# 3dhumangan/3DHumanGAN

Hardware: NVIDIA H100
Metric: images_per_sec_G_fwd_512x512 (higher is better)
Workload: dtype f32 (bf16x3 split on wgmma, fp32 accumulate)

## Files before the change

### 3dhumangan_b200/abi.py

```python
from __future__ import annotations

import ctypes
import os
from ctypes import c_char_p, c_double, c_float, c_int, c_long, c_size_t, c_void_p

import torch

_HERE = os.path.dirname(os.path.abspath(__file__))
LIB_PATH = os.path.join(_HERE, "lib3dhg_sm90a.so")
_lib = None

SIGNATURES = {
    "hg_last_error": (c_char_p, []),
    "hg_abi_version": (c_int, []),
    "hg_check_device": (c_int, []),
    "hg_packed_weight_bytes": (c_size_t, [c_int, c_int, c_int]),
    "hg_pack_weight": (c_int, [c_void_p, c_int, c_int, c_int, c_void_p, c_float, c_int, c_void_p, c_size_t, c_void_p]),
    "hg_vertex_ik": (c_int, [c_void_p, c_void_p, c_int, c_int, c_void_p, c_void_p]),
    "hg_knn_padded": (c_int, [c_int]),
    "hg_knn_prep": (c_int, [c_void_p, c_int, c_int, c_void_p, c_void_p, c_void_p]),
    "hg_geo_features": (c_int, [c_void_p] * 14 + [c_int] * 6 + [c_float, c_int] + [c_void_p] * 6),
    "hg_sample_fine": (c_int, [c_void_p, c_int, c_void_p, c_void_p, c_void_p, c_float, c_int] + [c_void_p] * 4 + [c_int] * 4
                       + [c_void_p] * 3),
    "hg_merge_samples": (c_int, [c_void_p] * 4 + [c_int] * 3 + [c_void_p] * 4),
    "hg_iso_workspace_bytes": (c_size_t, [c_int, c_int, c_int]),
    "hg_iso_count": (c_int, [c_void_p, c_int, c_int, c_int, c_float, c_void_p, c_size_t, c_void_p, c_void_p]),
    "hg_iso_emit": (c_int, [c_void_p, c_int, c_int, c_int] + [c_float] * 5 + [c_void_p, c_size_t, ctypes.c_longlong]
                    + [c_void_p] * 4),
    "hg_spade_conv": (c_int, [c_void_p, c_long, c_void_p, c_void_p, c_void_p, c_long] + [c_void_p] * 12 + [c_int] * 7 + [c_void_p]),
    "hg_bn_finalize": (c_int, [c_void_p, c_double, c_void_p, c_void_p, c_void_p, c_void_p, c_void_p, c_int, c_float, c_float,
                               c_void_p, c_int, c_int, c_void_p, c_void_p, c_void_p]),
    "hg_synth_input": (c_int, [c_void_p, c_void_p, c_void_p, c_void_p, c_int, c_int, c_int, c_void_p, c_void_p, c_int, c_void_p]),
    "hg_render_weight_blob_bytes": (c_size_t, []),
    "hg_render_mlp": (c_int, [c_void_p] * 12 + [c_int] * 4 + [c_float] + [c_int] * 4 + [c_void_p]),
    "hg_spade_bwd_dgrad": (c_int, [c_void_p, c_void_p, c_long, c_void_p, c_void_p, c_void_p, c_void_p] + [c_int] * 5 + [c_void_p]),
    "hg_spade_bwd_wgrad_workspace_bytes": (c_size_t, []),
    "hg_spade_bwd_wgrad": (c_int, [c_void_p, c_void_p, c_long, c_void_p, c_void_p, c_void_p, c_void_p] + [c_int] * 5 + [c_void_p]),
    "hg_spade_bwd_combine": (c_int, [c_void_p, c_void_p, c_long] + [c_void_p] * 7 + [c_int] * 4 + [c_void_p]),
    "hg_conv1x1_blocked": (c_int, [c_void_p, c_int, c_void_p, c_void_p, c_void_p] + [c_int] * 4 + [c_void_p]),
    "hg_conv1x1_blocked_bwd": (c_int, [c_void_p] * 7 + [c_int, c_float, c_int, c_int, c_void_p, c_void_p, c_void_p, c_int]
                               + [c_int] * 4 + [c_void_p]),
    "hg_act_conv1x1_blocked": (c_int, [c_void_p, c_void_p, c_void_p, c_int, c_void_p, c_void_p, c_void_p] + [c_int] * 4 + [c_void_p]),
    "hg_act_wgrad_blocked": (c_int, [c_void_p, c_void_p, c_void_p, c_long, c_int, c_void_p, c_int, c_void_p, c_void_p, c_void_p]
                             + [c_int] * 5 + [c_void_p]),
    "hg_render_heads": (c_int, [c_void_p] * 8 + [c_int, c_int, c_void_p]),
    "hg_render_heads_bwd": (c_int, [c_void_p] * 6 + [c_int, c_int, c_void_p]),
    "hg_render_composite": (c_int, [c_void_p] * 7 + [c_int, c_int, c_int, c_float, c_int, c_int, c_int, c_void_p]),
    "hg_blocked_conv_wide": (c_int, [c_void_p] * 4 + [c_int, c_float] + [c_void_p] * 9 + [c_int] * 4 + [c_void_p]),
    "hg_render_composite_bwd": (c_int, [c_void_p] * 9 + [c_int, c_int, c_int, c_float, c_int, c_int, c_int, c_void_p]),
    "hg_wgrad_blocked": (c_int, [c_void_p, c_void_p, c_long, c_int, c_void_p, c_void_p, c_void_p, c_void_p] + [c_int] * 5 + [c_void_p]),
    "hg_spade_a1": (c_int, [c_void_p, c_long, c_void_p, c_void_p] + [c_int] * 5 + [c_void_p]),
    "hg_spade_pixel_pre": (c_int, [c_void_p, c_long, c_void_p, c_void_p, c_void_p] + [c_int] * 4 + [c_void_p]),
    "hg_spade_pixel_mod_bwd": (c_int, [c_void_p, c_void_p, c_long, c_void_p, c_void_p, c_void_p, c_void_p] + [c_int] * 4 + [c_void_p]),
    "hg_bilinear_adjoint": (c_int, [c_void_p, c_void_p, c_long] + [c_int] * 5 + [c_void_p]),
    "hg_conv2d_wgrad_workspace_bytes": (c_size_t, []),
    "hg_conv2d_wgrad_taps": (c_int, [c_void_p] * 5 + [c_int] * 10 + [c_void_p, c_void_p, c_int, c_void_p]),
    "hg_conv2d_wgrad_layer_workspace_bytes": (c_size_t, [c_int] * 6),
    "hg_conv2d_wgrad_layer": (c_int, [c_void_p] * 5 + [c_size_t] + [c_int] * 7 + [c_void_p]),
    "hg_synth_input_bwd": (c_int, [c_void_p] * 5 + [c_int] * 4 + [c_void_p, c_void_p, c_void_p]),
    "hg_bias_act": (c_int, [c_void_p, c_void_p, c_void_p, c_long, c_int, c_int, c_int, c_float, c_float, c_float, c_void_p]),
    "hg_bias_act_grad": (c_int, [c_void_p] * 6 + [c_long, c_int, c_int, c_int, c_int, c_float, c_float, c_float, c_void_p]),
    "hg_resample2x": (c_int, [c_void_p, c_void_p, c_long, c_int, c_int, c_int, c_float, c_void_p]),
    "hg_upfirdn2d": (c_int, [c_void_p, c_void_p, c_void_p] + [c_int] * 14 + [c_float, c_void_p]),
    "hg_upfirdn2d_sep2": (c_int, [c_void_p, c_void_p, c_void_p, c_long] + [c_int] * 9 + [c_float, c_void_p]),
    "hg_conv2d": (c_int, [c_void_p, c_int, c_void_p, c_int] + [c_int] * 6 + [c_void_p, c_int, c_int, c_void_p, c_void_p, c_int,
                              c_void_p, c_int, c_void_p]),
    "hg_pool_add": (c_int, [c_void_p, c_int, c_void_p, c_int, c_void_p, c_long, c_int, c_int, c_void_p]),
    "hg_dense": (c_int, [c_void_p, c_void_p, c_void_p, c_void_p, c_int, c_int, c_int, c_void_p]),
    "hg_linear": (c_int, [c_void_p, c_int, c_int, c_int, c_void_p, c_int, c_int, c_void_p, c_void_p, c_int, c_int, c_void_p]),
    "hg_conv3x3_wgrad_halo_workspace_bytes": (ctypes.c_size_t, []),
    "hg_conv3x3_wgrad_halo": (c_int, [c_void_p] * 5 + [c_int] * 10 + [c_void_p, c_void_p, c_int, c_void_p]),
    "hg_label_histogram": (c_int, [c_void_p, c_long, c_int, c_void_p, c_void_p]),
    "hg_seg_ce_coef": (c_int, [c_void_p, c_void_p, c_int, c_double, c_void_p, c_void_p]),
    "hg_seg_ce": (c_int, [c_void_p] * 6 + [c_int, c_int, c_long, c_void_p]),
    "hg_image_loss": (c_int, [c_void_p] * 6 + [c_int, c_long, c_int, c_float, c_void_p]),
    "hg_latent_pool_gather": (c_int, [c_void_p, c_long, c_int, c_void_p, c_int, c_void_p, c_void_p]),
    "hg_latent_pool_grad": (c_int, [c_void_p, c_void_p, c_int, c_int, c_long, c_void_p, c_void_p]),
    "hg_latent_loss": (c_int, [c_void_p, c_void_p, c_int, c_int, c_float, c_void_p, c_void_p, c_void_p, c_void_p]),
    "hg_vgg_input": (c_int, [c_void_p, c_int, c_int, c_int, c_int, c_void_p, c_void_p, c_void_p, c_int, c_int, c_void_p]),
    "hg_vgg_input_adjoint": (c_int, [c_void_p, c_int, c_int, c_int, c_void_p, c_void_p, c_int, c_int, c_int, c_void_p]),
    "hg_maxpool2x2": (c_int, [c_void_p, c_void_p, c_long, c_int, c_int, c_void_p]),
    "hg_vgg_level_bwd": (c_int, [c_void_p] * 4 + [c_float, c_void_p, c_long, c_int, c_int, c_void_p]),
    "hg_smooth_l1": (c_int, [c_void_p, c_void_p, c_long, c_void_p, c_void_p, c_void_p]),
    "hg_conv2d_general": (c_int, [c_void_p] + [c_int] * 9 + [c_void_p, c_int, c_int, c_void_p, c_void_p, c_int, c_int, c_int,
                                                             c_void_p]),
    "hg_pool3x3": (c_int, [c_void_p] + [c_int] * 7 + [c_void_p, c_int, c_int, c_void_p]),
    "hg_global_avgpool": (c_int, [c_void_p, c_long, c_int, c_void_p, c_void_p]),
    "hg_feature_moments": (c_int, [c_void_p, c_int, c_int, c_void_p, c_void_p, c_void_p]),
    "hg_row_sqnorms": (c_int, [c_void_p, c_int, c_int, c_void_p, c_void_p]),
    "hg_knn_radii": (c_int, [c_void_p, c_void_p, c_int, c_int, c_int, c_void_p, c_void_p]),
    "hg_ball_coverage": (c_int, [c_void_p, c_void_p, c_void_p, c_int, c_void_p, c_void_p, c_void_p, c_int, c_int, c_void_p, c_void_p,
                                 c_void_p, c_void_p]),
    "hg_kid_workspace_bytes": (c_size_t, [c_int, c_int]),
    "hg_kid": (c_int, [c_void_p, c_int, c_void_p, c_int, c_int, c_void_p, c_void_p, c_int, c_int, c_void_p, c_void_p, c_size_t,
                       c_void_p]),
    "hg_mt_entry_bytes": (c_int, []),
    "hg_mt_chunk_bytes": (c_int, []),
    "hg_mt_chunk_elems": (c_int, []),
    "hg_mt_grad_norm": (c_int, [c_void_p, c_void_p, c_int, c_float, c_void_p, c_void_p, c_void_p]),
    "hg_mt_adam": (c_int, [c_void_p, c_void_p, c_int, c_void_p, c_void_p, c_int, c_float, c_int, c_void_p]),
    "hg_smpl_shape_blocks": (c_int, [c_int]),
    "hg_smpl_shape": (c_int, [c_void_p] * 6 + [c_int] * 4 + [c_void_p]),
    "hg_smpl_pose": (c_int, [c_void_p, c_int, c_void_p, c_int] + [c_void_p] * 6 + [c_int, c_int, c_void_p]),
    "hg_smpl_skin": (c_int, [c_void_p, c_long, c_void_p, c_void_p, c_int, c_void_p, c_long, c_void_p, c_void_p, c_int, c_int, c_int, c_void_p]),
    "hg_raster_project": (c_int, [c_void_p, c_void_p, c_void_p, c_float, c_void_p, c_int, c_int, c_void_p]),
    "hg_raster_faces": (c_int, [c_void_p, c_void_p] + [c_int] * 5 + [c_void_p, c_void_p]),
    "hg_raster_resolve": (c_int, [c_void_p] * 5 + [c_int] * 5 + [c_void_p] * 6),
    "hg_spectral_entry_bytes": (c_int, []),
    "hg_spectral_norm": (c_int, [c_void_p, c_int, c_int, c_int, c_void_p, c_int, c_float, c_void_p]),
}


def lib():
    global _lib
    if _lib is None:
        if not os.path.exists(LIB_PATH):
            raise RuntimeError(
# ... 495 lines not shown
```

### 3dhumangan_b200/csrc/render.cu

```cuda
#include "common.cuh"
#include "wgmma.cuh"

namespace hg {

constexpr int kRH = 256;
constexpr int kRenThreads = 384;
constexpr int kRenStages = 2;
constexpr uint32_t kRA = 128 * 128;
constexpr uint32_t kRB = 256 * 128;
constexpr int kFilmLayers = 7;
constexpr int kWeightStages = 60;
constexpr int kRayOut = 260;
constexpr int kScr = 65;

struct RenderArgs {
  const float* rec;
  const float* z_vals;
  const float* noise;
  const float* film;
  const uint8_t* wblob;
  const float* w_sigma;
  const float* w_rgb;
  const float* b_feat;
  const float* heads_b;
  float* ray_out;
  float* weights_out;
  float* raw_out;
  int B, R, S;
  float noise_std;
  int white_back, last_back, clamp_softplus;
};

struct RenSmem {
  uint8_t* a_hi;
  uint8_t* a_lo;
  uint8_t* b_st;
  float* film;
  float* w_sigma;
  float* w_rgb;
  float* b_feat;
  float* part;
  float* tr;
  float* wgt;
  float* zs;
  float* rayw;
  uint64_t* bars;
};
constexpr uint32_t kRenFloats = kFilmLayers * 2 * kRH + kRH + 3 * kRH + kRH + 128 * 4 + 4 * 128;
constexpr uint32_t kRenSmemBytes = 8 * kRA + kRenStages * kRB + kRenFloats * 4 + 16 * 8 + 1024;

__device__ __forceinline__ RenSmem ren_carve(uint8_t* raw) {
  uint8_t* s = reinterpret_cast<uint8_t*>((reinterpret_cast<uintptr_t>(raw) + 1023) & ~uintptr_t(1023));
  RenSmem m;
  m.a_hi = s;
  m.a_lo = s + 4 * kRA;
  m.b_st = s + 8 * kRA;
  float* f = reinterpret_cast<float*>(m.b_st + kRenStages * kRB);
  m.film = f; f += kFilmLayers * 2 * kRH;
  m.w_sigma = f; f += kRH;
  m.w_rgb = f; f += 3 * kRH;
  m.b_feat = f; f += kRH;
  m.part = f; f += 128 * 4;
  m.tr = f; f += 128;
  m.wgt = f; f += 128;
  m.zs = f; f += 128;
  m.rayw = f; f += 128;
  m.bars = reinterpret_cast<uint64_t*>(f);
  return m;
}
enum { RB_FULL = 0 , RB_EMPTY = 2  };

__device__ __forceinline__ void ren_rows_barrier() { named_barrier(1, 256); }

__device__ __forceinline__ float sin_reduced(float t) {
  const float y = t * 0.15915494309189535f;
  const float k = (y + 12582912.f) - 12582912.f;
  float r = fmaf(-k, 6.2831854820251465f, t);
  r = fmaf(-k, -1.7484555314695172e-07f, r);
  return __sinf(r);
}

__device__ __forceinline__ float2 sin_reduced2(float2 t) {
  const float2 y = fmul2(t, make_float2(0.15915494309189535f, 0.15915494309189535f));
  const float2 big = make_float2(12582912.f, 12582912.f), nbig = make_float2(-12582912.f, -12582912.f);
  const float2 k = fadd2(fadd2(y, big), nbig);
  float2 r = ffma2(k, make_float2(-6.2831854820251465f, -6.2831854820251465f), t);
  r = ffma2(k, make_float2(1.7484555314695172e-07f, 1.7484555314695172e-07f), r);
  return make_float2(__sinf(r.x), __sinf(r.y));
}

template <bool kSplit>
__device__ __forceinline__ void store_a2(uint8_t* tile_hi, uint8_t* tile_lo, uint32_t row, uint32_t k, float x0, float x1) {
  uint32_t h, l;
  split_bf16x2(x0, x1, h, l);
  const uint32_t off = sw128_offset(row, k);
  asm volatile("st.shared.b32 [%0], %1;" ::"r"(smem_u32(tile_hi) + off), "r"(h));
  if (kSplit) asm volatile("st.shared.b32 [%0], %1;" ::"r"(smem_u32(tile_lo) + off), "r"(l));
}

__device__ __forceinline__ void stash_store(float* slot, const float (&d)[128]) {
  const uint32_t base = static_cast<uint32_t>(__cvta_generic_to_local(slot));
#pragma unroll
  for (int i = 0; i < 128; i += 4)
    asm volatile("st.local.v4.f32 [%0], {%1, %2, %3, %4};" ::"r"(base + i * 4), "f"(d[i]), "f"(d[i + 1]), "f"(d[i + 2]), "f"(d[i + 3])
                 : "memory");
}
__device__ __forceinline__ float4 stash_load4(const float* slot, int i) {
  float4 v;
  asm volatile("ld.local.v4.f32 {%0, %1, %2, %3}, [%4];" : "=f"(v.x), "=f"(v.y), "=f"(v.z), "=f"(v.w)
               : "r"(static_cast<uint32_t>(__cvta_generic_to_local(slot)) + i * 4)
               : "memory");
  return v;
}

template <int kPasses, int kHead, bool kStash = false>
__device__ __forceinline__ void film_epilogue(const RenSmem& m, const float (&d)[128], const float* stash, int layer, int g, int t) {
  uint32_t F = smem_u32(m.film + (layer * 2 + 0) * kRH);
  uint32_t P = smem_u32(m.film + (layer * 2 + 1) * kRH);
  opaque(F);
  opaque(P);
  float dots[2][3] = {{0.f, 0.f, 0.f}, {0.f, 0.f, 0.f}};
#pragma unroll
  for (int j = 0; j < 32; ++j) {
    const int c = frag_col(t, j, 0);
    float f2[2], p2[2];
    asm("ld.shared.v2.f32 {%0, %1}, [%2];" : "=f"(f2[0]), "=f"(f2[1]) : "r"(F + c * 4));
    asm("ld.shared.v2.f32 {%0, %1}, [%2];" : "=f"(p2[0]), "=f"(p2[1]) : "r"(P + c * 4));
    float v[4] = {d[4 * j], d[4 * j + 1], d[4 * j + 2], d[4 * j + 3]};
    if (kStash) {
      const float4 q = stash_load4(stash, 4 * j);
      v[0] = q.x; v[1] = q.y; v[2] = q.z; v[3] = q.w;
    }
#pragma unroll
    for (int i = 0; i < 2; ++i) {
      const float2 x = sin_reduced2(ffma2(make_float2(f2[0], f2[1]), make_float2(v[2 * i], v[2 * i + 1]),
                                          make_float2(p2[0], p2[1])));
      if (kHead == 1) dots[i][0] = fmaf(x.y, m.w_sigma[c + 1], fmaf(x.x, m.w_sigma[c], dots[i][0]));
      if (kHead == 2) {
#pragma unroll
        for (int h = 0; h < 3; ++h) dots[i][h] = fmaf(x.y, m.w_rgb[h * kRH + c + 1], fmaf(x.x, m.w_rgb[h * kRH + c], dots[i][h]));
      }
      const int kc = c >> 6;
      store_a2<kPasses == 3>(m.a_hi + kc * kRA, m.a_lo + kc * kRA, g * 64 + frag_row(t, i), c & 63, x.x, x.y);
    }
  }
  if (kHead != 0) {
#pragma unroll
    for (int i = 0; i < 2; ++i) {
#pragma unroll
      for (int h = 0; h < 3; ++h) {
        if (kHead == 1 && h > 0) break;
        float v = dots[i][h];
        v += __shfl_xor_sync(0xffffffffu, v, 1);
        v += __shfl_xor_sync(0xffffffffu, v, 2);
        if ((t & 3) == 0) m.part[(g * 64 + frag_row(t, i)) * 4 + (kHead == 1 ? 0 : 1 + h)] = v;
      }
    }
  }
  fence_proxy_async_smem();
  named_barrier(2 + g, 128);
}

template <int kPasses>
__global__ void __launch_bounds__(kRenThreads, 1) render_mlp_kernel(RenderArgs a) {
  extern __shared__ uint8_t smem_raw[];
  const RenSmem m = ren_carve(smem_raw);
  const int warp = threadIdx.x >> 5, lane = threadIdx.x & 31;
  for (int i = threadIdx.x; i < kRH; i += blockDim.x) {
    m.w_sigma[i] = a.w_sigma[i];
    m.b_feat[i] = a.b_feat[i];
  }
  for (int i = threadIdx.x; i < 3 * kRH; i += blockDim.x) m.w_rgb[i] = a.w_rgb[i];
  if (threadIdx.x == 0) {
    for (int i = 0; i < kRenStages; ++i) {
      mbar_init(m.bars + RB_FULL + i, 1);
      mbar_init(m.bars + RB_EMPTY + i, 2);
    }
    fence_mbar_init();
  }
  __syncthreads();

  const int S = a.S;
  const int rpt = 128 / S;
  const int tiles_per_img = (a.R + rpt - 1) / rpt;
  const int num_tiles = a.B * tiles_per_img;
  const int my_tiles = (num_tiles - static_cast<int>(blockIdx.x) + static_cast<int>(gridDim.x) - 1) / static_cast<int>(gridDim.x);
  const long N = static_cast<long>(a.R) * S;

  if (warp < 8) {
    regs_inc<kMmaRegs>();
    const int g = warp >> 2, t = threadIdx.x & 127;
    const int tid = threadIdx.x;
    float d[128];
    __align__(16) float stash[128];
    uint32_t st = 0, ph = 0;
    uint32_t prev = ~0u;
    auto stage = [&](uint32_t a_tile, uint32_t a_tile2, bool two, bool accumulate) {
      mbar_wait(m.bars + RB_FULL + st, ph);
      acc_fence(d);
      wgmma_fence();
      const uint32_t bt = smem_u32(m.b_st + st * kRB);
      wg_k64<256>(d, a_tile, bt, accumulate);
      if (two) wg_k64<256>(d, a_tile2, bt, true);
      wgmma_commit();
      wgmma_wait<1>();
      acc_fence(d);
      if (prev != ~0u && t == 0) mbar_arrive(m.bars + RB_EMPTY + prev);
      prev = st;
      if (++st == kRenStages) { st = 0; ph ^= 1; }
    };
    auto layer = [&](int k0, int nk, bool accumulate) {
      for (int kc = k0; kc < k0 + nk; ++kc) {
        const uint32_t ahi = smem_u32(m.a_hi + kc * kRA) + g * 64 * 128, alo = smem_u32(m.a_lo + kc * kRA) + g * 64 * 128;
        stage(ahi, alo, kPasses == 3, accumulate || kc > k0);
        if (kPasses == 3) stage(ahi, ahi, false, true);
      }
      wgmma_wait<0>();
      acc_fence(d);
      if (t == 0) mbar_arrive(m.bars + RB_EMPTY + prev);
      prev = ~0u;
    };
    int cur_b = -1;
    for (int it = 0; it < my_tiles; ++it) {
      const int tile = blockIdx.x + it * gridDim.x;
      const int b = tile / tiles_per_img;
      const int ray0 = (tile % tiles_per_img) * rpt;
      if (b != cur_b) {
        ren_rows_barrier();
        for (int i = tid; i < kFilmLayers * 2 * kRH; i += 256)
          m.film[i] = a.film[static_cast<long>(b) * kFilmLayers * 2 * kRH + i];
        cur_b = b;
        ren_rows_barrier();
      }
      {
        const int row = g * 64 + (t >> 1), kh = t & 1;
        const int rl = row / S, s = row % S;
        const int ray = ray0 + rl;
        const bool valid = ray < a.R;
        const long gp = static_cast<long>(b) * N + static_cast<long>(ray) * S + s;
        float x[8];
        const float4* rp = reinterpret_cast<const float4*>(a.rec + gp * 36);
#pragma unroll
        for (int gi = 0; gi < 4; ++gi) {
          const int k0 = kh * 32 + gi * 8;
#pragma unroll
          for (int u = 0; u < 2; ++u) {
            const int f4 = (k0 >> 2) + u;
            float4 v = make_float4(0.f, 0.f, 0.f, 0.f);
            if (valid && f4 < 9) v = __ldg(rp + f4);
            x[u * 4 + 0] = v.x; x[u * 4 + 1] = v.y; x[u * 4 + 2] = v.z; x[u * 4 + 3] = v.w;
          }
          store_a8<kPasses == 3>(m.a_hi, m.a_lo, row, k0, x);
        }
        if (kh == 0) m.zs[row] = (valid && a.z_vals) ? a.z_vals[gp] : 0.f;
        fence_proxy_async_smem();
        named_barrier(2 + g, 128);
      }
      layer(0, 1, false);
      stash_store(stash, d);
      layer(0, 1, false);
      film_epilogue<kPasses, 0>(m, d, stash, 1, g, t);
      layer(0, 4, false);
      film_epilogue<kPasses, 0, true>(m, d, stash, 0, g, t);
      layer(0, 4, true);
      film_epilogue<kPasses, 0>(m, d, stash, 2, g, t);
      layer(0, 4, false);
      film_epilogue<kPasses, 0>(m, d, stash, 3, g, t);
      layer(0, 4, false);
      film_epilogue<kPasses, 0>(m, d, stash, 4, g, t);
      layer(0, 4, false);
      film_epilogue<kPasses, 1>(m, d, stash, 5, g, t);
      layer(0, 4, false);
      film_epilogue<kPasses, 2>(m, d, stash, 6, g, t);
      layer(0, 4, false);

      ren_rows_barrier();
      if (a.raw_out) {
        if (tid < 128) {
          const int row = tid, rl = row / S, s = row % S, ray = ray0 + rl;
          const long gp = static_cast<long>(b) * N + static_cast<long>(ray) * S + s;
          if (ray < a.R) {
            float* po = a.raw_out + gp * kRayOut;
            po[259] = m.part[row * 4] + a.heads_b[0];
            for (int j = 0; j < 3; ++j) {
              const float dot = m.part[row * 4 + 1 + j] + a.heads_b[1 + j];
              po[j] = 1.f / (1.f + expf(-dot));
            }
          }
        }
#pragma unroll
        for (int i = 0; i < 2; ++i) {
          const int row = g * 64 + frag_row(t, i), rl = row / S, s = row % S, ray = ray0 + rl;
// ... 25 lines not shown
      ren_rows_barrier();
      if (tid < 128) {
        const int row = tid, rl = row / S, s = row % S;
        float T = 1.f;
        for (int k = 0; k < s; ++k) T *= m.tr[rl * S + k];
        m.wgt[row] = ray0 + rl < a.R ? alpha * T : 0.f;
      }
      ren_rows_barrier();
      if (tid < rpt) {
        float W = 0.f;
        for (int k = 0; k < S; ++k) W += m.wgt[tid * S + k];
        m.rayw[tid] = W;
      }
      ren_rows_barrier();
      if (tid < 128) {
        const int row = tid, rl = row / S, s = row % S, ray = ray0 + rl;
        const float Wsum = m.rayw[rl];
        float w = m.wgt[row];
        const float w_depth = w + ((s == S - 1) ? 1.f - Wsum : 0.f);
        if (a.last_back) w = w_depth;
        if (a.weights_out && ray < a.R) a.weights_out[static_cast<long>(b) * N + static_cast<long>(ray) * S + s] = w;
        m.tr[row] = w;
        m.wgt[row] = w_depth;
      }
      ren_rows_barrier();

      float* scratch = reinterpret_cast<float*>(m.a_hi);
      const float wr[2] = {m.tr[g * 64 + frag_row(t, 0)], m.tr[g * 64 + frag_row(t, 1)]};
#pragma unroll
      for (int cg = 0; cg < 4; ++cg) {
#pragma unroll
        for (int i = 0; i < 2; ++i) {
          const int row = g * 64 + frag_row(t, i);
#pragma unroll
          for (int jj = 0; jj < 8; ++jj) {
            const int j = cg * 8 + jj, c = frag_col(t, j, 0);
            scratch[row * kScr + (c & 63)] = wr[i] * (d[4 * j + 2 * i] + m.b_feat[c]);
            scratch[row * kScr + (c & 63) + 1] = wr[i] * (d[4 * j + 2 * i + 1] + m.b_feat[c + 1]);
          }
        }
        ren_rows_barrier();
        {
          const int col = tid & 63;
          for (int r2 = tid >> 6; r2 < rpt; r2 += 4) {
            float acc = 0.f;
            const float* src = scratch + (r2 * S) * kScr + col;
            for (int k = 0; k < S; ++k) acc += src[k * kScr];
            if (ray0 + r2 < a.R)
              a.ray_out[(static_cast<long>(b) * a.R + ray0 + r2) * kRayOut + cg * 64 + col] =
                  acc + (a.white_back ? 1.f - m.rayw[r2] : 0.f);
          }
        }
        ren_rows_barrier();
      }
      if (tid < 128) {
        const int row = tid;
        const float w = m.tr[row];
#pragma unroll
        for (int j = 0; j < 3; ++j) {
          const float dot = m.part[row * 4 + 1 + j] + a.heads_b[1 + j];
          scratch[row * kScr + j] = w / (1.f + expf(-dot));
        }
        scratch[row * kScr + 3] = m.wgt[row] * m.zs[row];
      }
      ren_rows_barrier();
      if (tid < rpt && ray0 + tid < a.R) {
        float e[4] = {0.f, 0.f, 0.f, 0.f};
        for (int k = 0; k < S; ++k)
#pragma unroll
          for (int j = 0; j < 4; ++j) e[j] += scratch[(tid * S + k) * kScr + j];
        const float back = a.white_back ? 1.f - m.rayw[tid] : 0.f;
        float* ro = a.ray_out + (static_cast<long>(b) * a.R + ray0 + tid) * kRayOut;
        ro[256] = e[0] + back; ro[257] = e[1] + back; ro[258] = e[2] + back; ro[259] = e[3];
      }
      ren_rows_barrier();
    }
  } else {
    regs_dec<kProducerRegs>();
    if (warp == 8 && lane == 0) {
      uint32_t st = 0, ph = 0;
      for (int it = 0; it < my_tiles; ++it)
        for (int sidx = 0; sidx < kWeightStages; ++sidx) {
          if (kPasses == 1 && (sidx & 1)) continue;
          mbar_wait_backoff(m.bars + RB_EMPTY + st, ph ^ 1);
          mbar_arrive_expect_tx(m.bars + RB_FULL + st, kRB);
          bulk_g2s(m.b_st + st * kRB, a.wblob + static_cast<size_t>(sidx) * kRB, kRB, m.bars + RB_FULL + st);
          if (++st == kRenStages) { st = 0; ph ^= 1; }
        }
    }
  }
}

}

extern "C" {

size_t hg_render_weight_blob_bytes(void) { return static_cast<size_t>(hg::kWeightStages) * hg::kRB; }

int hg_render_mlp(const float* rec, const float* z_vals, const float* noise, const float* film, const void* wblob,
                  const float* w_sigma, const float* w_rgb, const float* b_feat, const float* heads_b, float* ray_out,
                  float* weights_out, float* raw_out, int B, int R, int S, int hidden, float noise_std, int white_back, int last_back,
                  int clamp_softplus, int passes, void* stream) {
  HG_REQUIRE(hidden == hg::kRH, "hg_render_mlp: only hidden_dim == %d is supported (got %d)", hg::kRH, hidden);
  HG_REQUIRE(rec && film && wblob && w_sigma && w_rgb && b_feat && heads_b, "hg_render_mlp: null pointer");
  HG_REQUIRE(raw_out || (ray_out && z_vals), "hg_render_mlp: need ray_out + z_vals (compositing) or raw_out (per-point)");
  HG_REQUIRE(B > 0 && R > 0, "hg_render_mlp: bad shape");
  HG_REQUIRE(S >= 2 && S <= 128 && (S & (S - 1)) == 0, "hg_render_mlp: samples per ray must be a power of two in [2,128] (got %d)", S);
  HG_REQUIRE(passes == 1 || passes == 3, "hg_render_mlp: passes must be 1 or 3");
  HG_REQUIRE((reinterpret_cast<uintptr_t>(rec) & 15) == 0 && (reinterpret_cast<uintptr_t>(wblob) & 15) == 0,
             "hg_render_mlp: rec / wblob must be 16-byte aligned");
  hg::RenderArgs a{rec, z_vals, noise, film, static_cast<const uint8_t*>(wblob), w_sigma, w_rgb, b_feat, heads_b,
                   ray_out, weights_out, raw_out, B, R, S, noise_std, white_back, last_back, clamp_softplus};
  const int rpt = 128 / S;
  const int tiles = B * ((R + rpt - 1) / rpt);
  const int grid = tiles < hg::num_sms() ? tiles : hg::num_sms();
  auto st = static_cast<cudaStream_t>(stream);
  cudaError_t e;
  if (passes == 3) {
    e = cudaFuncSetAttribute(hg::render_mlp_kernel<3>, cudaFuncAttributeMaxDynamicSharedMemorySize, hg::kRenSmemBytes);
    if (e != cudaSuccess) { hg::set_error("hg_render_mlp: smem opt-in failed: %s", cudaGetErrorString(e)); return 2; }
    hg::render_mlp_kernel<3><<<grid, hg::kRenThreads, hg::kRenSmemBytes, st>>>(a);
  } else {
    e = cudaFuncSetAttribute(hg::render_mlp_kernel<1>, cudaFuncAttributeMaxDynamicSharedMemorySize, hg::kRenSmemBytes);
    if (e != cudaSuccess) { hg::set_error("hg_render_mlp: smem opt-in failed: %s", cudaGetErrorString(e)); return 2; }
    hg::render_mlp_kernel<1><<<grid, hg::kRenThreads, hg::kRenSmemBytes, st>>>(a);
  }
  return hg::check_launch("hg_render_mlp");
}

}
```

### 3dhumangan_b200/csrc/wgmma.cuh

```cuda
#pragma once
#include <cuda_bf16.h>
#include <cuda_runtime.h>
#include <stdint.h>

#include "common.cuh"

namespace hg {

__device__ __forceinline__ uint32_t smem_u32(const void* p) {
  return static_cast<uint32_t>(__cvta_generic_to_shared(p));
}

__device__ __forceinline__ void mbar_init(uint64_t* bar, uint32_t count) {
  asm volatile("mbarrier.init.shared::cta.b64 [%0], %1;" ::"r"(smem_u32(bar)), "r"(count) : "memory");
}
__device__ __forceinline__ void fence_mbar_init() {
  asm volatile("fence.mbarrier_init.release.cluster;" ::: "memory");
}
__device__ __forceinline__ void mbar_arrive(uint64_t* bar) {
  asm volatile("mbarrier.arrive.shared::cta.b64 _, [%0];" ::"r"(smem_u32(bar)) : "memory");
}
__device__ __forceinline__ void mbar_arrive_expect_tx(uint64_t* bar, uint32_t bytes) {
  asm volatile("mbarrier.arrive.expect_tx.shared::cta.b64 _, [%0], %1;" ::"r"(smem_u32(bar)), "r"(bytes) : "memory");
}
__device__ __forceinline__ bool mbar_try_wait(uint64_t* bar, uint32_t parity) {
  uint32_t ok;
  asm volatile(
      "{\n\t.reg .pred p;\n\t"
      "mbarrier.try_wait.parity.shared::cta.b64 p, [%1], %2;\n\t"
      "selp.u32 %0, 1, 0, p;\n\t}"
      : "=r"(ok)
      : "r"(smem_u32(bar)), "r"(parity)
      : "memory");
  return ok != 0;
}
__device__ __forceinline__ void mbar_wait(uint64_t* bar, uint32_t parity) {
  while (!mbar_try_wait(bar, parity)) {
  }
}
__device__ __forceinline__ void mbar_wait_sleep(uint64_t* bar, uint32_t parity) {
  while (!mbar_try_wait(bar, parity)) __nanosleep(32);
}
__device__ __forceinline__ void mbar_wait_backoff(uint64_t* bar, uint32_t parity) {
  while (!mbar_try_wait(bar, parity)) __nanosleep(128);
}

__device__ __forceinline__ void named_barrier(uint32_t id, uint32_t n) {
  asm volatile("bar.sync %0, %1;" ::"r"(id), "r"(n) : "memory");
}

template <uint32_t kRegs>
__device__ __forceinline__ void regs_inc() { asm volatile("setmaxnreg.inc.sync.aligned.u32 %0;" ::"n"(kRegs)); }
template <uint32_t kRegs>
__device__ __forceinline__ void regs_dec() { asm volatile("setmaxnreg.dec.sync.aligned.u32 %0;" ::"n"(kRegs)); }
constexpr uint32_t kMmaRegs = 232, kProducerRegs = 40;

__device__ __forceinline__ float lds_f32(uint32_t addr) {
  float v;
  asm volatile("ld.shared.f32 %0, [%1];" : "=f"(v) : "r"(addr));
  return v;
}
__device__ __forceinline__ void sts_b32x4(uint32_t addr, uint32_t a, uint32_t b, uint32_t c, uint32_t d) {
  asm volatile("st.shared.v4.b32 [%0], {%1, %2, %3, %4};" ::"r"(addr), "r"(a), "r"(b), "r"(c), "r"(d));
}
__device__ __forceinline__ void opaque(uint32_t& r) { asm volatile("" : "+r"(r)); }
__device__ __forceinline__ void lds8(uint32_t a, float (&o)[8]) {
  float4 x, y;
  asm("ld.shared.v4.f32 {%0, %1, %2, %3}, [%4];" : "=f"(x.x), "=f"(x.y), "=f"(x.z), "=f"(x.w) : "r"(a));
  asm("ld.shared.v4.f32 {%0, %1, %2, %3}, [%4];" : "=f"(y.x), "=f"(y.y), "=f"(y.z), "=f"(y.w) : "r"(a + 16));
  o[0] = x.x; o[1] = x.y; o[2] = x.z; o[3] = x.w;
  o[4] = y.x; o[5] = y.y; o[6] = y.z; o[7] = y.w;
}

__device__ __forceinline__ void fence_proxy_async_smem() {
  asm volatile("fence.proxy.async.shared::cta;" ::: "memory");
}

__device__ __forceinline__ void bulk_g2s(void* smem_dst, const void* gmem_src, uint32_t bytes, uint64_t* bar) {
  asm volatile("cp.async.bulk.shared::cluster.global.mbarrier::complete_tx::bytes [%0], [%1], %2, [%3];" ::"r"(
                   smem_u32(smem_dst)),
               "l"(gmem_src), "r"(bytes), "r"(smem_u32(bar))
               : "memory");
}

__device__ __forceinline__ uint64_t wg_desc_sw128(uint32_t smem_addr) {
  uint64_t d = 0;
  d |= static_cast<uint64_t>((smem_addr >> 4) & 0x3FFF);
  d |= static_cast<uint64_t>(1) << 16;
  d |= static_cast<uint64_t>(1024 >> 4) << 32;
  d |= static_cast<uint64_t>(1) << 62;
  return d;
}

template <int N, int kTransB = 0>
__device__ __forceinline__ void wgmma_bf16(float (&d)[N / 2], uint64_t da, uint64_t db, uint32_t accumulate);

#define HG_ACC4(i) "+f"(d[i]), "+f"(d[i + 1]), "+f"(d[i + 2]), "+f"(d[i + 3])
#define HG_ACC16(i) HG_ACC4(i), HG_ACC4(i + 4), HG_ACC4(i + 8), HG_ACC4(i + 12)
#define HG_ACC32 HG_ACC16(0), HG_ACC16(16)
#define HG_ACC64 HG_ACC32, HG_ACC16(32), HG_ACC16(48)
#define HG_ACC128 HG_ACC64, HG_ACC16(64), HG_ACC16(80), HG_ACC16(96), HG_ACC16(112)
#define HG_REGS32 \
  "%0, %1, %2, %3, %4, %5, %6, %7, %8, %9, %10, %11, %12, %13, %14, %15, " \
  "%16, %17, %18, %19, %20, %21, %22, %23, %24, %25, %26, %27, %28, %29, %30, %31"
#define HG_REGS64 \
  HG_REGS32 ", %32, %33, %34, %35, %36, %37, %38, %39, %40, %41, %42, %43, %44, %45, %46, %47, " \
  "%48, %49, %50, %51, %52, %53, %54, %55, %56, %57, %58, %59, %60, %61, %62, %63"
#define HG_REGS128 \
  HG_REGS64 ", %64, %65, %66, %67, %68, %69, %70, %71, %72, %73, %74, %75, %76, %77, %78, %79, " \
  "%80, %81, %82, %83, %84, %85, %86, %87, %88, %89, %90, %91, %92, %93, %94, %95, " \
  "%96, %97, %98, %99, %100, %101, %102, %103, %104, %105, %106, %107, %108, %109, %110, %111, " \
  "%112, %113, %114, %115, %116, %117, %118, %119, %120, %121, %122, %123, %124, %125, %126, %127"
#define HG_WGMMA(kN, kTransB, NREG, REGS, ACC, DA, FLAG)                                                        \
  template <>                                                                                                 \
  __device__ __forceinline__ void wgmma_bf16<kN, kTransB>(float (&d)[NREG], uint64_t da, uint64_t db,          \
                                                          uint32_t accumulate) {                              \
    asm volatile("{\n\t.reg .pred p;\n\tsetp.ne.b32 p, " FLAG ", 0;\n\t"                                     \
                 "wgmma.mma_async.sync.aligned.m64n" #kN "k16.f32.bf16.bf16 {" REGS "}, " DA ", p, 1, 1, 0, " #kTransB \
                 ";\n\t}"                                                                                    \
                 : ACC                                                                                        \
                 : "l"(da), "l"(db), "r"(accumulate));                                                        \
  }
HG_WGMMA(64, 0, 32, HG_REGS32, HG_ACC32, "%32, %33", "%34")
HG_WGMMA(128, 0, 64, HG_REGS64, HG_ACC64, "%64, %65", "%66")
HG_WGMMA(256, 0, 128, HG_REGS128, HG_ACC128, "%128, %129", "%130")
HG_WGMMA(64, 1, 32, HG_REGS32, HG_ACC32, "%32, %33", "%34")
#undef HG_WGMMA

__device__ __forceinline__ void wgmma_fence() { asm volatile("wgmma.fence.sync.aligned;" ::: "memory"); }
__device__ __forceinline__ void wgmma_commit() { asm volatile("wgmma.commit_group.sync.aligned;" ::: "memory"); }
template <int kPending>
__device__ __forceinline__ void wgmma_wait() {
  asm volatile("wgmma.wait_group.sync.aligned %0;" ::"n"(kPending) : "memory");
}
template <int kN>
__device__ __forceinline__ void acc_fence(float (&d)[kN]) {
#pragma unroll
  for (int i = 0; i < kN; ++i) asm volatile("" : "+f"(d[i])::"memory");
}

template <int N>
__device__ __forceinline__ void wg_k64(float (&d)[N / 2], uint32_t a_tile, uint32_t b_tile, bool accumulate) {
  const uint64_t da = wg_desc_sw128(a_tile);
  const uint64_t db = wg_desc_sw128(b_tile);
#pragma unroll
  for (uint32_t k = 0; k < 4; ++k) {
    wgmma_bf16<N>(d, da + 2 * k, db + 2 * k, (accumulate || k > 0) ? 1u : 0u);
  }
}

__device__ __forceinline__ int frag_row(int t, int i) { return ((t >> 5) << 4) + ((t & 31) >> 2) + 8 * i; }
__device__ __forceinline__ int frag_col(int t, int j, int e) { return 8 * j + 2 * (t & 3) + e; }

__host__ __device__ __forceinline__ uint32_t sw128_offset(uint32_t row, uint32_t k) {
  return (row >> 3) * 1024u + (row & 7u) * 128u + ((((k >> 3) ^ row) & 7u) << 4) + ((k & 7u) << 1);
}

__device__ __forceinline__ void split_bf16x2(float x0, float x1, uint32_t& hi, uint32_t& lo) {
  __nv_bfloat162 h = __floats2bfloat162_rn(x0, x1);
  const uint32_t hb = *reinterpret_cast<uint32_t*>(&h);
  const float2 hf = make_float2(__uint_as_float(hb << 16), __uint_as_float(hb & 0xffff0000u));
  const float2 r = ffma2(hf, make_float2(-1.f, -1.f), make_float2(x0, x1));
  __nv_bfloat162 l = __floats2bfloat162_rn(r.x, r.y);
  hi = hb;
  lo = *reinterpret_cast<uint32_t*>(&l);
// ... 27 lines not shown
```

### include/hg3d.h

```cpp
#ifndef HG3D_H_
#define HG3D_H_

#include <stddef.h>

#ifdef __cplusplus
extern "C" {
#endif

const char* hg_last_error(void);
int hg_abi_version(void);
int hg_check_device(void);

size_t hg_packed_weight_bytes(int N, int K, int Nb);
int hg_pack_weight(const float* W, int N, int K, int ldw, const float* scale_dev, float scale, int Nb,
                   void* out_img, size_t out_bytes, void* stream);

int hg_linear(const float* X, int ldx, int M, int K, const void* Wimg, int Nb, int N, const float* bias, float* Y,
              int ldy, int passes, void* stream);

int hg_vertex_ik(const float* fk, const float* lbs, int B, int V, float* vertex_ik, void* stream);

int hg_knn_padded(int V);
int hg_knn_prep(const float* vertices, int B, int V, void* sorted, void* boxes, void* stream);

int hg_geo_features(const float* xs, const float* ys, const float* zs, const float* focals, const float* scales,
                    const float* cam2world, const float* jitter, const float* points_in, const float* skeletons,
                    const float* vertices, const float* tpose, const float* vertex_ik, const void* knn_sorted,
                    const void* knn_boxes, int B, int Rw, int Rh, int S, int V, int n_points, float input_scaler,
                    int legacy_mode, float* rec, float* z_vals, float* points, int* nearest, float* nearest_d2,
                    void* stream);

int hg_sample_fine(const float* sigma, int sigma_stride, const float* z_vals, const float* noise, const float* u_pdf,
                   float noise_std, int clamp_softplus, const float* xs, const float* ys, const float* focals,
                   const float* cam2world, int B, int Rw, int Rh, int S, float* fine_z, float* fine_points, void* stream);

int hg_merge_samples(const float* fine_rec, const float* fine_z, const float* coarse_rec, const float* coarse_z, int B,
                     int R, int S, float* rec_out, float* z_out, int* perm_out, void* stream);

size_t hg_render_weight_blob_bytes(void);
int hg_render_mlp(const float* rec, const float* z_vals, const float* noise, const float* film, const void* wblob,
                  const float* w_sigma, const float* w_rgb, const float* b_feat, const float* heads_b, float* ray_out,
                  float* weights_out, float* raw_out, int B, int R, int S, int hidden, float noise_std, int white_back,
                  int last_back, int clamp_softplus, int passes, void* stream);

size_t hg_iso_workspace_bytes(int nz, int ny, int nx);
int hg_iso_count(const float* lattice, int nz, int ny, int nx, float level, void* workspace, size_t workspace_bytes,
                 long long* totals, void* stream);
int hg_iso_emit(const float* lattice, int nz, int ny, int nx, float ox, float oy, float oz, float spacing, float level,
                const void* workspace, size_t workspace_bytes, long long n_vertices, float* vertices, float* normals, int* faces,
                void* stream);

int hg_synth_input(const float* w, const float* bias, const float* ic, const float* jc, int C, int Hg, int Wg,
                   float* x0, double* stats, int batch, void* stream);

int hg_bn_finalize(const double* stats, double count, const double* count_dev, const float* weight, const float* bias,
                   float* running_mean, float* running_var, int training, float eps, float momentum, const float* gb,
                   int B, int C, float* scsh, float* mod, void* stream);

int hg_spade_conv(const float* x, long x_bstride, const float* mod, const float* scsh, const float* p_lr,
                  long p_stride, const float* p_bias, const void* wgb, const float* bgb, const void* wimg,
                  const float* bias, const float* skip, float* out, double* stats, const float* rgb_w,
                  const float* rgb_b, const float* rgb_in, float* rgb_out, int B, int C, int Hg, int Wg, int Rh, int Rw,
                  int passes, void* stream);

int hg_spade_bwd_dgrad(const float* dout, const float* x, long x_bstride, const float* mod, const void* wimg_t,
                       float* dpre, double* sums, int B, int C, int Hg, int Wg, int passes, void* stream);
size_t hg_spade_bwd_wgrad_workspace_bytes(void);
int hg_spade_bwd_wgrad(const float* dout, const float* x, long x_bstride, const float* mod, float* dw, float* dbias,
                       void* workspace, int B, int C, int Hg, int Wg, int passes, void* stream);
int hg_conv1x1_blocked(const float* x, int Cin, const void* wimg, const float* bias, float* out, int B, int Hg, int Wg,
                       int passes, void* stream);
int hg_conv1x1_blocked_bwd(const float* g, const float* g2, const float* aux, const float* mod, const void* wimg_t,
                           float* out, double* sums, int Cout, float slope, int pixel_major, int act, const float* ascale,
                           const float* rk_w, const float* rk_v, int rk_n, int B, int Hg, int Wg, int passes,
                           void* stream);
int hg_act_conv1x1_blocked(const float* x, const float* x2, const float* mod, int act, const void* wimg, const float* bias,
                           float* out, int B, int Hg, int Wg, int passes, void* stream);
int hg_blocked_conv_wide(const float* x, const float* x2, const float* mod, const float* mod2, int act, float slope,
                         const void* wimg, const float* bias, const float* skip, float* out, double* stats,
                         const float* rgb_w, const float* rgb_b, const float* rgb_in, float* rgb_out, int B, int Hg, int Wg,
                         int passes, void* stream);
int hg_act_wgrad_blocked(const float* dout, const float* pscale, const float* x, long x_bstride, int Cx, const float* mod,
                         int act, float* dw, float* dbias, void* workspace, int B, int C, int Hg, int Wg, int passes,
                         void* stream);
int hg_render_heads(const float* out3, const float* linc, const float* mod3, const float* w_sigma, const float* w_rgb,
                    const float* heads_b, float* sig, float* rgbp, int B, int N, void* stream);
int hg_render_heads_bwd(const float* out3, const float* linc, const float* mod3, const float* dsig, const float* drgbp,
                        double* acc, int B, int N, void* stream);
int hg_render_composite(const float* sig, const float* z, const float* noise, const float* rgbp, const float* feat,
                        float* ray_out, float* weights, int B, int R, int S, float noise_std, int white_back,
                        int clamp_softplus, int last_back, void* stream);
int hg_render_composite_bwd(const float* sig, const float* z, const float* noise, const float* rgbp, const float* feat,
                            const float* dray, float* dfeat, float* drgbp, float* dsig, int B, int R, int S,
                            float noise_std, int white_back, int clamp_softplus, int last_back, void* stream);
int hg_wgrad_blocked(const float* dout, const float* x, long x_bstride, int Cx, const float* mod, float* dw, float* dbias,
                     void* workspace, int B, int C, int Hg, int Wg, int passes, void* stream);
int hg_spade_a1(const float* p_lr, long p_stride, const float* p_bias, float* a1, int B, int Hg, int Wg, int Rh, int Rw,
                void* stream);
int hg_spade_pixel_pre(const float* x, long x_bstride, const float* scsh, const float* gam, float* bet_pre, int B, int C,
                       int Hg, int Wg, void* stream);
int hg_spade_pixel_mod_bwd(const float* dpre, const float* x, long x_bstride, const float* scsh, float* gam_dgam, float* dxn,
                           double* sums, int B, int C, int Hg, int Wg, void* stream);
int hg_bilinear_adjoint(const float* da1, float* dp, long dp_stride, int B, int Hg, int Wg, int Rh, int Rw, void* stream);

size_t hg_conv2d_wgrad_workspace_bytes(void);
int hg_conv2d_wgrad_taps(const float* dy, const float* x, float* dw, float* dbias, void* workspace, int B, int H, int W,
                         int Cout, int Cin, int co0, int nco, int ci0, int nci, int ntaps, const int* oy, const int* ox,
                         int passes, void* stream);
size_t hg_conv2d_wgrad_layer_workspace_bytes(int B, int H, int W, int Cout, int Cin, int ksize);
int hg_conv2d_wgrad_layer(const float* dy, const float* x, float* dW, float* dbias, void* workspace, size_t workspace_bytes, int B,
                          int H, int W, int Cout, int Cin, int ksize, int passes, void* stream);
size_t hg_conv3x3_wgrad_halo_workspace_bytes(void);
int hg_conv3x3_wgrad_halo(const float* dy, const float* x, float* dw, float* dbias, void* workspace, int B, int H, int W,
                          int Cout, int Cin, int co0, int nco, int ci0, int nci, int ntaps, const int* tdy, const int* tdx,
                          int passes, void* stream);
int hg_synth_input_bwd(const float* dx, const float* w, const float* bias, const float* ic, const float* jc, int B, int C,
                       int Hg, int Wg, float* dw, float* db, void* stream);
int hg_spade_bwd_combine(const float* dpre, const float* x, long x_bstride, const float* g1, const float* ak,
                         const float* dskip, const float* drgb, const float* rgb_w, float* dx, double* dwrgb, int B,
                         int C, int Hg, int Wg, void* stream);


int hg_conv2d(const float* x1, int C1, const float* x2, int C2, int B, int H, int W, int up2, int pre_lrelu, int ksize,
              const void* wimg, int Cout, int Nb, const float* bias, const float* residual, int res_up2, float* out,
              int passes, void* stream);
int hg_pool_add(const float* a, int pool_a, const float* b, int pool_b, float* out, long planes, int H, int W,
// ... 81 lines not shown
```

Baseline: 99.96.

## Split render MLP weight stages into half-width slots for finer TMA pipelining

For the three-pass bf16 split path, each 32 KB weight stage is now delivered as two 16 KB half-N slots in a four-slot ring, and wgmma runs N=128 per half. The aim is finer-grained overlap between the bulk weight copies and the matmuls, so compute can start on half a stage before the rest has landed. The cost is twice as many mbarrier waits and commits and smaller wgmma shapes. A separate standalone L2 bulk/multicast copy probe kernel is also added for measurement and is not called from the forward path.

```diff
diff --git a/3dhumangan_b200/abi.py b/3dhumangan_b200/abi.py
--- a/3dhumangan_b200/abi.py
+++ b/3dhumangan_b200/abi.py
@@ -33,6 +33,7 @@
     "hg_synth_input": (c_int, [c_void_p, c_void_p, c_void_p, c_void_p, c_int, c_int, c_int, c_void_p, c_void_p, c_int, c_void_p]),
     "hg_render_weight_blob_bytes": (c_size_t, []),
     "hg_render_mlp": (c_int, [c_void_p] * 12 + [c_int] * 4 + [c_float] + [c_int] * 4 + [c_void_p]),
+    "hg_l2_bulk_probe": (c_int, [c_void_p, c_size_t, c_int, c_int, c_void_p, c_void_p]),
     "hg_spade_bwd_dgrad": (c_int, [c_void_p, c_void_p, c_long, c_void_p, c_void_p, c_void_p, c_void_p] + [c_int] * 5 + [c_void_p]),
     "hg_spade_bwd_wgrad_workspace_bytes": (c_size_t, []),
     "hg_spade_bwd_wgrad": (c_int, [c_void_p, c_void_p, c_long, c_void_p, c_void_p, c_void_p, c_void_p] + [c_int] * 5 + [c_void_p]),
diff --git a/3dhumangan_b200/csrc/render.cu b/3dhumangan_b200/csrc/render.cu
--- a/3dhumangan_b200/csrc/render.cu
+++ b/3dhumangan_b200/csrc/render.cu
@@ -5,9 +5,11 @@
 
 constexpr int kRH = 256;
 constexpr int kRenThreads = 384;
-constexpr int kRenStages = 2;
 constexpr uint32_t kRA = 128 * 128;
 constexpr uint32_t kRB = 256 * 128;
+constexpr uint32_t kRenRing = 2 * kRB;
+template <int kPasses>
+constexpr int ren_parts() { return kPasses == 3 ? 2 : 1; }
 constexpr int kFilmLayers = 7;
 constexpr int kWeightStages = 60;
 constexpr int kRayOut = 260;
@@ -47,7 +49,7 @@
   uint64_t* bars;
 };
 constexpr uint32_t kRenFloats = kFilmLayers * 2 * kRH + kRH + 3 * kRH + kRH + 128 * 4 + 4 * 128;
-constexpr uint32_t kRenSmemBytes = 8 * kRA + kRenStages * kRB + kRenFloats * 4 + 16 * 8 + 1024;
+constexpr uint32_t kRenSmemBytes = 8 * kRA + kRenRing + kRenFloats * 4 + 16 * 8 + 1024;
 
 __device__ __forceinline__ RenSmem ren_carve(uint8_t* raw) {
   uint8_t* s = reinterpret_cast<uint8_t*>((reinterpret_cast<uintptr_t>(raw) + 1023) & ~uintptr_t(1023));
@@ -55,7 +57,7 @@
   m.a_hi = s;
   m.a_lo = s + 4 * kRA;
   m.b_st = s + 8 * kRA;
-  float* f = reinterpret_cast<float*>(m.b_st + kRenStages * kRB);
+  float* f = reinterpret_cast<float*>(m.b_st + kRenRing);
   m.film = f; f += kFilmLayers * 2 * kRH;
   m.w_sigma = f; f += kRH;
   m.w_rgb = f; f += 3 * kRH;
@@ -68,7 +70,7 @@
   m.bars = reinterpret_cast<uint64_t*>(f);
   return m;
 }
-enum { RB_FULL = 0 , RB_EMPTY = 2  };
+enum { RB_FULL = 0 , RB_EMPTY = 4  };
 
 __device__ __forceinline__ void ren_rows_barrier() { named_barrier(1, 256); }
 
@@ -163,6 +165,8 @@
 
 template <int kPasses>
 __global__ void __launch_bounds__(kRenThreads, 1) render_mlp_kernel(RenderArgs a) {
+  constexpr int kParts = ren_parts<kPasses>(), kSlots = 2 * kParts;
+  constexpr uint32_t kSlot = kRB / kParts;
   extern __shared__ uint8_t smem_raw[];
   const RenSmem m = ren_carve(smem_raw);
   const int warp = threadIdx.x >> 5, lane = threadIdx.x & 31;
@@ -172,7 +176,7 @@
   }
   for (int i = threadIdx.x; i < 3 * kRH; i += blockDim.x) m.w_rgb[i] = a.w_rgb[i];
   if (threadIdx.x == 0) {
-    for (int i = 0; i < kRenStages; ++i) {
+    for (int i = 0; i < kSlots; ++i) {
       mbar_init(m.bars + RB_FULL + i, 1);
       mbar_init(m.bars + RB_EMPTY + i, 2);
     }
@@ -196,18 +200,23 @@
     uint32_t st = 0, ph = 0;
     uint32_t prev = ~0u;
     auto stage = [&](uint32_t a_tile, uint32_t a_tile2, bool two, bool accumulate) {
-      mbar_wait(m.bars + RB_FULL + st, ph);
-      acc_fence(d);
-      wgmma_fence();
-      const uint32_t bt = smem_u32(m.b_st + st * kRB);
-      wg_k64<256>(d, a_tile, bt, accumulate);
-      if (two) wg_k64<256>(d, a_tile2, bt, true);
-      wgmma_commit();
-      wgmma_wait<1>();
-      acc_fence(d);
-      if (prev != ~0u && t == 0) mbar_arrive(m.bars + RB_EMPTY + prev);
-      prev = st;
-      if (++st == kRenStages) { st = 0; ph ^= 1; }
+      constexpr int kN = kRH / kParts;
+#pragma unroll
+      for (int h = 0; h < kParts; ++h) {
+        float(&dh)[kN / 2] = *reinterpret_cast<float(*)[kN / 2]>(d + kN / 2 * h);
+        mbar_wait(m.bars + RB_FULL + st, ph);
+        acc_fence(d);
+        wgmma_fence();
+        const uint32_t bt = smem_u32(m.b_st + st * kSlot);
+        wg_k64<kN>(dh, a_tile, bt, accumulate);
+        if (two) wg_k64<kN>(dh, a_tile2, bt, true);
+        wgmma_commit();
+        wgmma_wait<1>();
+        acc_fence(d);
+        if (prev != ~0u && t == 0) mbar_arrive(m.bars + RB_EMPTY + prev);
+        prev = st;
+        if (++st == kSlots) { st = 0; ph ^= 1; }
+      }
     };
     auto layer = [&](int k0, int nk, bool accumulate) {
       for (int kc = k0; kc < k0 + nk; ++kc) {
@@ -399,13 +408,58 @@
       for (int it = 0; it < my_tiles; ++it)
         for (int sidx = 0; sidx < kWeightStages; ++sidx) {
           if (kPasses == 1 && (sidx & 1)) continue;
-          mbar_wait_backoff(m.bars + RB_EMPTY + st, ph ^ 1);
-          mbar_arrive_expect_tx(m.bars + RB_FULL + st, kRB);
-          bulk_g2s(m.b_st + st * kRB, a.wblob + static_cast<size_t>(sidx) * kRB, kRB, m.bars + RB_FULL + st);
-          if (++st == kRenStages) { st = 0; ph ^= 1; }
-        }
-    }
-  }
+          for (uint32_t h = 0; h < kParts; ++h) {
+            mbar_wait_backoff(m.bars + RB_EMPTY + st, ph ^ 1);
+            mbar_arrive_expect_tx(m.bars + RB_FULL + st, kSlot);
+            bulk_g2s(m.b_st + st * kSlot, a.wblob + static_cast<size_t>(sidx) * kRB + h * kSlot, kSlot, m.bars + RB_FULL + st);
+            if (++st == kSlots) { st = 0; ph ^= 1; }
+          }
+        }
+    }
+  }
+}
+
+constexpr int kProbeCluster = 2, kProbeSlots = 4;
+constexpr uint32_t kProbeSlot = 16384, kProbeShare = kProbeSlot / kProbeCluster;
+
+__global__ void __launch_bounds__(64, 1) bulk_probe_kernel(const uint8_t* src, int src_slots, int slots, int multicast) {
+  extern __shared__ uint8_t smem_raw[];
+  uint8_t* buf = reinterpret_cast<uint8_t*>((reinterpret_cast<uintptr_t>(smem_raw) + 1023) & ~uintptr_t(1023));
+  uint64_t* bars = reinterpret_cast<uint64_t*>(buf + kProbeSlots * kProbeSlot);
+  if (threadIdx.x == 0) {
+    for (int i = 0; i < kProbeSlots; ++i) {
+      mbar_init(bars + i, 1);
+      mbar_init(bars + kProbeSlots + i, multicast ? kProbeCluster : 1);
+    }
+    fence_mbar_init();
+  }
+  cluster_sync();
+  const uint32_t rank = cluster_ctarank();
+  uint32_t st = 0, ph = 0;
+  if (threadIdx.x == 0) {
+    for (int s = 0; s < slots; ++s) {
+      const uint8_t* from = src + static_cast<size_t>((s + blockIdx.x / kProbeCluster) % src_slots) * kProbeSlot;
+      mbar_wait_backoff(bars + kProbeSlots + st, ph ^ 1);
+      mbar_arrive_expect_tx(bars + st, kProbeSlot);
+      if (multicast)
+        bulk_g2s_multicast(buf + st * kProbeSlot + rank * kProbeShare, from + rank * kProbeShare, kProbeShare, bars + st,
+                           (1u << kProbeCluster) - 1);
+      else
+        bulk_g2s(buf + st * kProbeSlot, from, kProbeSlot, bars + st);
+      if (++st == kProbeSlots) { st = 0; ph ^= 1; }
+    }
+  } else if (threadIdx.x == 32) {
+    for (int s = 0; s < slots; ++s) {
+      mbar_wait(bars + st, ph);
+      if (multicast)
+        for (uint32_t r = 0; r < kProbeCluster; ++r) mbar_arrive_cluster(bars + kProbeSlots + st, r);
+      else
+        mbar_arrive(bars + kProbeSlots + st);
+      if (++st == kProbeSlots) { st = 0; ph ^= 1; }
+    }
+  }
+  __syncwarp();
+  cluster_sync();
 }
 
 }
@@ -445,4 +499,32 @@
   return hg::check_launch("hg_render_mlp");
 }
 
-}
+int hg_l2_bulk_probe(const void* src, size_t src_bytes, int slots, int multicast, int* ctas, void* stream) {
+  HG_REQUIRE(src && (reinterpret_cast<uintptr_t>(src) & 15) == 0, "hg_l2_bulk_probe: src must be 16-byte aligned");
+  HG_REQUIRE(src_bytes >= hg::kProbeSlot && slots > 0 && ctas, "hg_l2_bulk_probe: need at least one 16 KB slot and ctas");
+  cudaError_t e = cudaFuncSetAttribute(hg::bulk_probe_kernel, cudaFuncAttributeMaxDynamicSharedMemorySize, hg::kRenSmemBytes);
+  if (e != cudaSuccess) { hg::set_error("hg_l2_bulk_probe: smem opt-in failed: %s", cudaGetErrorString(e)); return 2; }
+  cudaLaunchAttribute attr[1];
+  attr[0].id = cudaLaunchAttributeClusterDimension;
+  attr[0].val.clusterDim.x = hg::kProbeCluster;
+  attr[0].val.clusterDim.y = 1;
+  attr[0].val.clusterDim.z = 1;
+  cudaLaunchConfig_t cfg = {};
+  cfg.gridDim = dim3(hg::kProbeCluster * hg::num_sms());
+  cfg.blockDim = dim3(64);
+  cfg.dynamicSmemBytes = hg::kRenSmemBytes;
+  cfg.stream = static_cast<cudaStream_t>(stream);
+  cfg.attrs = attr;
+  cfg.numAttrs = 1;
+  int clusters = 0;
+  e = cudaOccupancyMaxActiveClusters(&clusters, hg::bulk_probe_kernel, &cfg);
+  if (e != cudaSuccess || clusters <= 0) { hg::set_error("hg_l2_bulk_probe: no resident cluster: %s", cudaGetErrorString(e)); return 2; }
+  cfg.gridDim = dim3(hg::kProbeCluster * clusters);
+  *ctas = hg::kProbeCluster * clusters;
+  e = cudaLaunchKernelEx(&cfg, hg::bulk_probe_kernel, static_cast<const uint8_t*>(src), static_cast<int>(src_bytes / hg::kProbeSlot),
+                         slots, multicast);
+  if (e != cudaSuccess) { hg::set_error("hg_l2_bulk_probe: launch failed: %s", cudaGetErrorString(e)); return 2; }
+  return hg::check_launch("hg_l2_bulk_probe");
+}
+
+}
diff --git a/3dhumangan_b200/csrc/wgmma.cuh b/3dhumangan_b200/csrc/wgmma.cuh
--- a/3dhumangan_b200/csrc/wgmma.cuh
+++ b/3dhumangan_b200/csrc/wgmma.cuh
@@ -45,6 +45,23 @@
   while (!mbar_try_wait(bar, parity)) __nanosleep(128);
 }
 
+__device__ __forceinline__ uint32_t cluster_ctarank() {
+  uint32_t r;
+  asm volatile("mov.u32 %0, %%cluster_ctarank;" : "=r"(r));
+  return r;
+}
+__device__ __forceinline__ void cluster_sync() {
+  asm volatile("barrier.cluster.arrive.release.aligned;\n\tbarrier.cluster.wait.acquire.aligned;" ::: "memory");
+}
+__device__ __forceinline__ void mbar_arrive_cluster(uint64_t* bar, uint32_t rank) {
+  asm volatile(
+      "{\n\t.reg .b32 ra;\n\t"
+      "mapa.shared::cluster.u32 ra, %0, %1;\n\t"
+      "mbarrier.arrive.release.cluster.shared::cluster.b64 _, [ra];\n\t}" ::"r"(smem_u32(bar)),
+      "r"(rank)
+      : "memory");
+}
+
 __device__ __forceinline__ void named_barrier(uint32_t id, uint32_t n) {
   asm volatile("bar.sync %0, %1;" ::"r"(id), "r"(n) : "memory");
 }
@@ -81,6 +98,14 @@
                    smem_u32(smem_dst)),
                "l"(gmem_src), "r"(bytes), "r"(smem_u32(bar))
                : "memory");
+}
+__device__ __forceinline__ void bulk_g2s_multicast(void* smem_dst, const void* gmem_src, uint32_t bytes, uint64_t* bar,
+                                                   uint16_t cta_mask) {
+  asm volatile(
+      "cp.async.bulk.shared::cluster.global.mbarrier::complete_tx::bytes.multicast::cluster [%0], [%1], %2, [%3], %4;" ::"r"(
+          smem_u32(smem_dst)),
+      "l"(gmem_src), "r"(bytes), "r"(smem_u32(bar)), "h"(cta_mask)
+      : "memory");
 }
 
 __device__ __forceinline__ uint64_t wg_desc_sw128(uint32_t smem_addr) {
diff --git a/include/hg3d.h b/include/hg3d.h
--- a/include/hg3d.h
+++ b/include/hg3d.h
@@ -42,6 +42,7 @@
                   const float* w_sigma, const float* w_rgb, const float* b_feat, const float* heads_b, float* ray_out,
                   float* weights_out, float* raw_out, int B, int R, int S, int hidden, float noise_std, int white_back,
                   int last_back, int clamp_softplus, int passes, void* stream);
+int hg_l2_bulk_probe(const void* src, size_t src_bytes, int slots, int multicast, int* ctas, void* stream);
 
 size_t hg_iso_workspace_bytes(int nz, int ny, int nx);
 int hg_iso_count(const float* lattice, int nz, int ny, int nx, float level, void* workspace, size_t workspace_bytes,
```

Result: faster. 102.0, median of 6 (+2.0%).
